# Samleo8/RadarSLAMPy

Measured on AMD Instinct MI355X. Metric: radar scan-pairs/sec (400x3768 polar), higher is better.
Workload: dtype u8/f32/f64

## Files before the change

radarslampy_amd/csrc/engine.hip:

```cpp
#include "roam_internal.h"
#include "retrack.h"
#include "kabsch_body.inc"
#include <algorithm>
#include <new>

#define KS ROAM_MAX_FEATURES
#define CART_CENTER 1012.0
#define M_PER_PX 0.0864
#define N_RETRACK 60
#define ROT_THR 0.2
#define TRANS_THR_SQ 4.0
#define ERR_THR 10.0f
#define TWO_PI 6.283185307179586476925286766559

#define RES_RING 8
enum { ST_PEAKS = 0, ST_WARP, ST_PYR, ST_KLT, ST_GRAPH, ST_CLIQUE, ST_KABSCH, ST_LM, ST_GLUE, ST_RETRACK, ST_COUNT };
static const char *kStageNames[ST_COUNT] = {"ingest_peaks", "warp_quantise", "pyramid", "klt", "consistency_graph",
                                            "max_clique", "kabsch", "mds_lm", "glue", "retrack"};

struct Engine {
    roam_engine_cfg cfg;
    int B = 0, W = 0, stage_cap = 0;
    PyrDesc pd;
    size_t rec_bytes = 0;
// ... 35 lines not shown
    int lm_big_slot = 0;
    roam_lane_result *results = nullptr;
    roam_lane_result *results_host = nullptr;
    hipEvent_t ev_res[8] = {nullptr, nullptr, nullptr, nullptr, nullptr, nullptr, nullptr, nullptr};
    hipEvent_t ev_pool = nullptr;
    bool pool_dirty = false;
    RtArgs rt;
    bool rt_on = false;
    int rt_mode = 1;
    uint8_t *kfb = nullptr;
    uint8_t *rmap = nullptr;
    int rmap_cap = 0;
    int64_t rmap_n = 0;
    int64_t rmap_n_bcast = 0;
    std::vector<int32_t> rmap_root;
    uint8_t *kfx_send = nullptr, *kfx_recv = nullptr;
    size_t kfx_rec = 0;
    int kfx_peaks = 0;
    int kfx_world = 0;
    int64_t *rmap_n_dev = nullptr;
    int32_t *rmap_root_dev = nullptr;
    int64_t kfx_calls = 0;
    bool kfx_ready = false;
    hipStream_t st_comm = nullptr;
    hipEvent_t ev_kfx[3] = {};
    int kfx_last = -1;
    hipEvent_t ev[ST_COUNT + 1] = {};
    bool stage_ev_forced = false;
    bool stage_ev = true;
    hipEvent_t ev_join = nullptr, ev_pk0 = nullptr, ev_pk1 = nullptr;
    hipEvent_t ev_klt[4] = {}, ev_g4[4] = {};
    hipEvent_t ev_warp = nullptr;
    hipEvent_t ev_idx = nullptr, ev_peaks = nullptr;
    hipEvent_t tr_ev[64][6] = {};
    hipEvent_t rt_ev[64][3 * RT_TRACE_CHUNKS] = {};
    bool rt_ev_ok[64] = {};
    hipEvent_t ev_emit = nullptr;
    RtSide det_side = {};
    int det_chunk() const { return (det_side.chunk > 0 && retrack_sided(rt, B, &det_side)) ? det_side.chunk : rt.slots; }
    int64_t rt_image_px = 0;
    bool tr_ev_ok[64] = {};
    int64_t stage_ev_step = -1;
    bool tr_ok = false;
    unsigned long long *pyr_dark = nullptr;
    static constexpr bool warp_dark_zero = true;
    bool ev_ok = false, stepped = false, uploads_pending = false;
    uint64_t up_seq = 0, up_waited = 0;
    std::vector<uint64_t> slot_seq;
    hipEvent_t ev_up_ring[16] = {};
    std::vector<int> lane_k;
    int rt_floor = 320;
    int kmax() const { int m = rt_on ? rt_floor : 64; for (int k : lane_k) m = k > m ? k : m; m = (m + 63) & ~63; return m > KS ? KS : m; }
    std::vector<void *> allocs;
};

template <typename T>
static bool dalloc(roam_ctx *ctx, Engine *e, T **p, size_t count)
{
    void *q = nullptr;
    size_t bytes = count * sizeof(T);
    if (bytes == 0) bytes = 16;
    hipError_t err = hipMalloc(&q, bytes);
    if (err != hipSuccess) {
        ROAM_SET_ERR(ctx, "engine: hipMalloc(%zu) failed: %s", bytes, hipGetErrorString(err));
        return false;
    }
// ... 135 lines not shown
        Ti[3] = s * ko[0] + c * ko[2]; Ti[4] = s * ko[1] + c * ko[3]; Ti[5] = s * hx + c * hy + y;
        Ti[6] = 0; Ti[7] = 0; Ti[8] = 1;
    }
}


#define MAP_SLOT (8 + 2 * KS)
__device__ __forceinline__ void map_freeze(double *__restrict__ map_store, int32_t *__restrict__ map_n, int map_cap, int b,
                                           const double *__restrict__ kfp, const double *__restrict__ kfv, int n,
                                           int scan, const double *__restrict__ locals)
{
    const int slot = map_n[b];
    if (slot >= map_cap) return;
    double *d = map_store + ((size_t)b * map_cap + slot) * MAP_SLOT;
    for (int j = threadIdx.x; j < 2 * n; j += blockDim.x) d[8 + j] = locals[j];
    if (threadIdx.x == 0) {
        d[0] = kfp[0]; d[1] = kfp[1]; d[2] = kfp[2];
        d[3] = kfv[0]; d[4] = kfv[1]; d[5] = kfv[2];
        d[6] = (double)n; d[7] = (double)scan;
    }
}

__global__ __launch_bounds__(256) void map_freeze_kernel(double *__restrict__ map_store, int32_t *__restrict__ map_n, int map_cap,
                                                         int b, const double *__restrict__ kf_pose,
                                                         const double *__restrict__ kf_vel, const int32_t *__restrict__ feat_n,
                                                         const int32_t *__restrict__ kf_scan, const double *__restrict__ kf_und,
                                                         const int32_t *__restrict__ kf_live, const int32_t *__restrict__ kf_fresh)
{
    if (!kf_live[b] || kf_fresh[b]) return;
    const int slot = map_n[b];
    map_freeze(map_store, map_n, map_cap, b, kf_pose + 3 * b, kf_vel + 3 * b, feat_n[b], kf_scan[b], kf_und + (size_t)b * KS * 2);
    __syncthreads();
    if (threadIdx.x == 0 && slot < map_cap) map_n[b] = slot + 1;
}

__global__ __launch_bounds__(256) void g4_update_kernel(roam_engine_cfg cfg, const double *__restrict__ lm_out,
                                                        const int32_t *__restrict__ lm_nfev, const int32_t *__restrict__ lm_info,
                                                        const double *__restrict__ kab_out, double *__restrict__ pose,
                                                        double *__restrict__ vel, double *__restrict__ kf_pose,
                                                        double *__restrict__ kf_und, const double *__restrict__ kf_und_tmp,
                                                        const double *__restrict__ p_jt, const int32_t *__restrict__ in_n,
                                                        const int32_t *__restrict__ good_n, int32_t *__restrict__ feat_n,
                                                        const int32_t *__restrict__ peaks_n, const int32_t *__restrict__ cq_flags,
                                                        roam_lane_result *__restrict__ res, const int32_t *__restrict__ scan_idx,
                                                        double *__restrict__ kf_vel, int32_t *__restrict__ kf_scan,
                                                        int32_t *__restrict__ kf_fresh, const int32_t *__restrict__ kf_live,
                                                        double *__restrict__ map_store, int32_t *__restrict__ map_n, int map_cap,
                                                        int collect, int32_t *__restrict__ rt_lane, int32_t *__restrict__ rt_scan,
                                                        int32_t *__restrict__ rt_n)
{
    __shared__ double np_[3], nv_[3];
    __shared__ int newkf;
    const int b = blockIdx.x, t = threadIdx.x;
    const int n = in_n[b];
    if (t == 0) {
        double px = pose[3 * b], py = pose[3 * b + 1], pth = pose[3 * b + 2];
        double v0 = 0, v1 = 0, v2 = 0;
        const double *k = kab_out + 6 * (int64_t)b;
        if (n >= 2) {
            if (cfg.motion_distortion) {
                const double *s = lm_out + 6 * (int64_t)b;
                v0 = s[0]; v1 = s[1]; v2 = s[2]; px = s[3]; py = s[4]; pth = s[5];
            } else {
                const double dx = k[4] * M_PER_PX, dy = k[5] * M_PER_PX, dth = atan2(k[2], k[0]);
                const double c = cos(pth), s = sin(pth);
                px += dx * c - dy * s; py += dx * s + dy * c; pth += dth;
// ... 25 lines not shown
        if (newkf) {
            const double x = p_jt[2 * o], y = p_jt[2 * o + 1];
            const double dT = 0.25 * atan2(-y, -x) / TWO_PI;
            const double a = v2 * dT, ca = cos(a), sa = sin(a);
            kf_und[2 * o] = ca * x - sa * y + v0 * dT;
            kf_und[2 * o + 1] = sa * x + ca * y + v1 * dT;
        } else {
            kf_und[2 * o] = kf_und_tmp[2 * o]; kf_und[2 * o + 1] = kf_und_tmp[2 * o + 1];
        }
    }
    __syncthreads();
    if (t == 0) {
        pose[3 * b] = np_[0]; pose[3 * b + 1] = np_[1]; pose[3 * b + 2] = np_[2];
        vel[3 * b] = v0; vel[3 * b + 1] = v1; vel[3 * b + 2] = v2;
        if (newkf) {
            kf_pose[3 * b] = np_[0]; kf_pose[3 * b + 1] = np_[1]; kf_pose[3 * b + 2] = np_[2];
            kf_vel[3 * b] = v0; kf_vel[3 * b + 1] = v1; kf_vel[3 * b + 2] = v2;
            kf_scan[b] = scan_idx[b];
            if (mslot >= 0 && mslot < map_cap) map_n[b] = mslot + 1;
        }
        kf_fresh[b] = newkf;
        feat_n[b] = n;
    }
    if (collect) {
        __shared__ int last_s, sh[4], base_s;
#if defined(__HIP_DEVICE_COMPILE__) && !defined(__gfx942__) && !defined(__gfx950__)
#error "g4_update_kernel's hand-off to its last block relies on gfx94x/95x storing with write-through and counting stores in vmcnt: s_waitcnt vmcnt(0) + relaxed atomics, no release/acquire pair"
#endif
        asm volatile("s_waitcnt vmcnt(0)" ::: "memory");
        __syncthreads();
        if (t == 0) last_s = atomicAdd(rt_n + 1, 1) == (int)gridDim.x - 1;
        __syncthreads();
        if (!last_s) return;
        const int B = (int)gridDim.x;
        if (t == 0) base_s = 0;
        __syncthreads();
        for (int b0 = 0; b0 < B; b0 += 256) {
            const int bb = b0 + t;
            const int f = (bb < B && (collect == 2 || (__hip_atomic_load(&res[bb].flags, __ATOMIC_RELAXED, __HIP_MEMORY_SCOPE_AGENT) & 4))) ? 1 : 0;
            const int lane = t & 63, w = t >> 6;
            int inc = f;
#pragma unroll
            for (int d = 1; d < 64; d <<= 1) { const int nn = __shfl_up(inc, d); if (lane >= d) inc += nn; }
            if (lane == 63) sh[w] = inc;
            __syncthreads();
            int off = base_s, tot = 0;
            for (int i = 0; i < 4; i++) { if (i < w) off += sh[i]; tot += sh[i]; }
            if (f) { rt_lane[off + inc - 1] = bb; rt_scan[off + inc - 1] = scan_idx[bb]; }
            __syncthreads();
            if (t == 0) base_s += tot;
            __syncthreads();
        }
        if (t == 0) { rt_n[0] = base_s; rt_n[1] = 0; }
    }
}

__global__ void lane_kf_reset_kernel(const float *__restrict__ feat, int K, const double *__restrict__ vel,
                                     double *__restrict__ kf_und)
{
    const int j = blockIdx.x * blockDim.x + threadIdx.x;
    if (j >= K) return;
    const double x = ((double)feat[2 * j] - CART_CENTER) * M_PER_PX, y = ((double)feat[2 * j + 1] - CART_CENTER) * M_PER_PX;
    const double dT = 0.25 * atan2(-y, -x) / TWO_PI;
    const double a = vel[2] * dT, ca = cos(a), sa = sin(a);
    kf_und[2 * j] = ca * x - sa * y + vel[0] * dT;
    kf_und[2 * j + 1] = sa * x + ca * y + vel[1] * dT;
}

#define KFB_HDR 64
#define KFB_LOCALS_OFF KFB_HDR
#define KFB_PEAKS_OFF (KFB_HDR + KS * 16)
__global__ __launch_bounds__(256) void kf_pack_kernel(uint8_t *__restrict__ buf, int lane, const double *__restrict__ kf_pose,
                                                      const double *__restrict__ kf_vel, const int32_t *__restrict__ feat_n,
                                                      const int32_t *__restrict__ kf_scan, const double *__restrict__ kf_und,
                                                      const int32_t *__restrict__ peaks_n, const int32_t *__restrict__ peaks,
                                                      int peaks_cap)
{
    const int t = blockIdx.x * blockDim.x + threadIdx.x, nt = gridDim.x * blockDim.x;
    int n = feat_n[lane], P = peaks_n[lane];
    if (n > KS) n = KS;
    if (P > peaks_cap) P = peaks_cap;
    if (t == 0) {
        roam_keyframe_hdr *h = reinterpret_cast<roam_keyframe_hdr *>(buf);
        for (int i = 0; i < 3; i++) { h->pose[i] = kf_pose[3 * lane + i]; h->velocity[i] = kf_vel[3 * lane + i]; }
        h->n_features = n; h->n_peaks = P; h->scan = kf_scan[lane]; h->lane = lane;
// ... 56 lines not shown
    }
    __syncthreads();
    if (threadIdx.x == 0) *n_dev = cnt;
}

typedef uint32_t u32x4_a1 __attribute__((ext_vector_type(4), aligned(1)));
__global__ __launch_bounds__(256) void ingest_rows_kernel(const uint8_t *__restrict__ host, int64_t host_stride, uint8_t *__restrict__ pool,
                                                          int64_t rec_bytes, int rows, int stride, int width)
{
    const int rec = blockIdx.y, row = blockIdx.x * 4 + (threadIdx.x >> 6), lane = threadIdx.x & 63;
    if (row >= rows) return;
    const uint8_t *s = host + (int64_t)rec * host_stride + (int64_t)row * stride;
    uint8_t *d = pool + (int64_t)rec * rec_bytes + (int64_t)row * stride;
    const int nvec = width / 16;
    for (int v = lane; v < nvec; v += 64) *reinterpret_cast<u32x4_a1 *>(d + 16 * v) = *reinterpret_cast<const u32x4_a1 *>(s + 16 * v);
    for (int b = nvec * 16 + lane; b < width; b += 64) d[b] = s[b];
}

extern "C" {

int32_t roam_engine_destroy(roam_ctx *ctx)
{
    if (!ctx) return ROAM_E_ARG;
    Engine *e = ctx->engine;
    if (!e) return ROAM_OK;
    hipSetDevice(ctx->device);
    hipStreamSynchronize(ctx->stream);
    for (void *p : e->allocs) hipFree(p);
    auto kill = [](hipEvent_t &ev) { if (ev) { hipEventDestroy(ev); ev = nullptr; } };
    for (auto &ev : e->ev) kill(ev);
    for (int i = 0; i < 4; i++) { kill(e->det_side.ev_i[i]); kill(e->det_side.ev_d[i]); }
    kill(e->ev_emit);
    kill(e->ev_join); kill(e->ev_pk0); kill(e->ev_pk1); kill(e->ev_warp); kill(e->ev_idx); kill(e->ev_peaks);
    for (int i = 0; i < 4; i++) { kill(e->ev_klt[i]); kill(e->ev_g4[i]); }
    for (auto &row : e->tr_ev) for (auto &ev : row) kill(ev);
    for (auto &row : e->rt_ev) for (auto &ev : row) kill(ev);
    if (e->scan_host) hipHostFree(e->scan_host);
    if (e->results_host) hipHostFree(e->results_host);
    for (auto &ev : e->ev_res) if (ev) hipEventDestroy(ev);
    if (e->st_comm) { hipStreamSynchronize(e->st_comm); hipStreamDestroy(e->st_comm); }
    for (auto &ev : e->ev_kfx) if (ev) hipEventDestroy(ev);
    if (e->ev_pool) hipEventDestroy(e->ev_pool);
    for (auto &ev : e->ev_up_ring) if (ev) hipEventDestroy(ev);
    hipStreamSynchronize(ctx->stream2);
    hipStreamSynchronize(ctx->stream4);
    delete e;
    ctx->engine = nullptr;
    return ROAM_OK;
}

static int32_t fused_tables(roam_ctx *ctx, Engine *e)
{
    RtArgs &r = e->rt;
    if (r.fd_mapT) return ROAM_OK;
    const size_t npx = (size_t)e->W * e->W, R = (size_t)r.slots;
    uint32_t *mapT = nullptr, *boxtab = nullptr, *darktab = nullptr;
    bool ok = dalloc(ctx, e, &mapT, npx) && dalloc(ctx, e, &boxtab, retrack_fused_boxtab_words(e->W)) && dalloc(ctx, e, &darktab, retrack_darktab_words(e->W));
    ok = ok && dalloc(ctx, e, &r.fd_halo, R * 2 * (size_t)r.fd_halo_words) && dalloc(ctx, e, &r.fd_cc, R * 2048);
    if (!ok) return ROAM_E_HIP;
    HIP_TRY(ctx, launch_retrack_fused_tables(ctx->stream, e->warp_map, e->W, e->cfg.clip, mapT, boxtab, darktab));
    HIP_TRY(ctx, hipStreamSynchronize(ctx->stream));
    r.fd_boxtab = boxtab; r.fd_darktab = darktab;
    r.fd_mapT = mapT;
    return ROAM_OK;
}

// ... 106 lines not shown
        }
        const size_t D = (size_t)B;
        ok = ok && dalloc(ctx, e, &r.cand_rc, D * BP_MAX_PTS) && dalloc(ctx, e, &r.cand_val, D * BP_MAX_PTS) && dalloc(ctx, e, &r.cand_n, D);
        ok = ok && dalloc(ctx, e, &r.tasks, D * BP_MAX_TASKS) && dalloc(ctx, e, &r.pairs, D * (BP_MAX_PAIRS + 1));
        ok = ok && dalloc(ctx, e, &r.order, D * (BP_MAX_PAIRS + 1)) && dalloc(ctx, e, &r.ovbits, D * ((BP_MAX_PAIRS + 31) / 32 + 1));
        ok = ok && dalloc(ctx, e, &r.bigtab, D * 2 * 131072);
        ok = ok && dalloc(ctx, e, &r.kp, D * BP_MAX_PTS * 3) && dalloc(ctx, e, &r.kp_n, D) && dalloc(ctx, e, &r.slot_flags, D);
        ok = ok && dalloc(ctx, e, &r.ssc_work, D * 4 * BP_MAX_PTS) && dalloc(ctx, e, &r.sel, D * BP_MAX_PTS) && dalloc(ctx, e, &r.sel_n, D) && dalloc(ctx, e, &r.blob_order_buf, D);
    }
    if (!ok) { roam_engine_destroy(ctx); return ROAM_E_HIP; }
    if (e->rt_on) {
        if (hipError_t er = retrack_init(); er != hipSuccess) {
            ROAM_SET_ERR(ctx, "retrack_init failed: %s", hipGetErrorString(er));
            roam_engine_destroy(ctx);
            return ROAM_E_HIP;
        }
        RtArgs &r = e->rt;
        r.pool = e->pool; r.map = e->warp_map; r.feat = e->feat; r.feat_n = e->feat_n; r.vel = e->vel; r.kf_und = e->kf_und; r.res = nullptr;
    }
    for (auto &ev : e->ev_res)
        if (hipEventCreateWithFlags(&ev, hipEventDisableTiming) != hipSuccess) { ROAM_SET_ERR(ctx, "hipEventCreate failed"); roam_engine_destroy(ctx); return ROAM_E_HIP; }
    e->slot_seq.assign((size_t)cfg->pool_scans, 0);
    for (auto &ev : e->ev_up_ring)
        if (hipEventCreateWithFlags(&ev, hipEventDisableTiming) != hipSuccess) { ROAM_SET_ERR(ctx, "hipEventCreate failed"); roam_engine_destroy(ctx); return ROAM_E_HIP; }
    if (hipEventCreateWithFlags(&e->ev_pool, hipEventDisableTiming) != hipSuccess) {
        ROAM_SET_ERR(ctx, "hipEventCreate failed"); roam_engine_destroy(ctx); return ROAM_E_HIP;
    }
    for (auto &ev : e->ev) {
        if (hipEventCreate(&ev) != hipSuccess) { ROAM_SET_ERR(ctx, "hipEventCreate failed"); roam_engine_destroy(ctx); return ROAM_E_HIP; }
    }
    if (hipEventCreate(&e->ev_join) != hipSuccess ||
        hipEventCreate(&e->ev_pk0) != hipSuccess || hipEventCreate(&e->ev_pk1) != hipSuccess ||
        hipEventCreateWithFlags(&e->ev_warp, hipEventDisableTiming) != hipSuccess || hipEventCreateWithFlags(&e->ev_idx, hipEventDisableTiming) != hipSuccess ||
        hipEventCreateWithFlags(&e->ev_peaks, hipEventDisableTiming) != hipSuccess) {
        ROAM_SET_ERR(ctx, "hipEventCreate failed"); roam_engine_destroy(ctx); return ROAM_E_HIP;
    }
    for (int i = 0; i < 4; i++)
        if (hipEventCreateWithFlags(&e->ev_klt[i], hipEventDisableTiming) != hipSuccess || hipEventCreateWithFlags(&e->ev_g4[i], hipEventDisableTiming) != hipSuccess) {
            ROAM_SET_ERR(ctx, "hipEventCreate failed"); roam_engine_destroy(ctx); return ROAM_E_HIP;
        }
    e->ev_ok = true;
    e->tr_ok = true;
    HIP_TRY(ctx, launch_warp_map(ctx->stream, cfg->rows, cfg->clip, e->warp_map));
    HIP_TRY(ctx, launch_pyr_dark(ctx->stream, e->warp_map, e->W, e->W, cfg->clip, e->pyr_dark));
    if (e->rt_on) HIP_TRY(ctx, launch_retrack_boxtab(ctx->stream, e->warp_map, e->W, cfg->clip, const_cast<uint32_t *>(e->rt.boxtab)));
    if (e->rt_on) HIP_TRY(ctx, launch_retrack_darktab(ctx->stream, e->warp_map, e->W, cfg->clip, const_cast<uint32_t *>(e->rt.darktab)));
    if (e->rt_on && e->rt.fused) { const int32_t rc_ = fused_tables(ctx, e); if (rc_ != ROAM_OK) { roam_engine_destroy(ctx); return rc_; } }
    HIP_TRY(ctx, hipStreamSynchronize(ctx->stream));
    e->rt_image_px = (int64_t)e->W * e->W;
    if (e->rt_on && e->W <= 2048 && B >= RT_TWO_PASS_SLOTS) {
        e->rt_image_px = 0;
        const size_t npx = (size_t)e->W * e->W, ndt = retrack_darktab_words(e->W), nph = retrack_phase_words(e->W);
        uint32_t *stage = nullptr;
        HIP_TRY(ctx, hipHostMalloc(reinterpret_cast<void **>(&stage), (npx + ndt + nph) * 4, hipHostMallocDefault));
        uint32_t *mh = stage, *dh = stage + npx;
        std::vector<uint32_t> ph(nph, 0u);
        hipError_t ec = hipMemcpyAsync(mh, e->warp_map, npx * 4, hipMemcpyDeviceToHost, ctx->stream);
        if (ec == hipSuccess) ec = hipMemcpyAsync(dh, e->rt.darktab, ndt * 4, hipMemcpyDeviceToHost, ctx->stream);
        if (ec == hipSuccess) ec = hipStreamSynchronize(ctx->stream);
        bool okp = ec == hipSuccess && retrack_build_phases(mh, dh, e->W, cfg->clip, ph.data());
        if (okp) {
            memcpy(stage + npx + ndt, ph.data(), nph * 4);
            ec = hipMemcpyAsync(const_cast<uint32_t *>(e->rt.phlist), stage + npx + ndt, nph * 4, hipMemcpyHostToDevice, ctx->stream);
            if (ec == hipSuccess) ec = hipStreamSynchronize(ctx->stream);
        }
        (void)hipHostFree(stage);
        if (!okp || ec != hipSuccess) { ROAM_SET_ERR(ctx, "retrack: phase list (%s)", ec != hipSuccess ? hipGetErrorString(ec) : "image too large"); roam_engine_destroy(ctx); return ec != hipSuccess ? ROAM_E_HIP : ROAM_E_ARG; }
// ... 492 lines not shown
    HIP_TRY(ctx, hipEventRecord(e->ev_warp, sA));
    HIP_TRY(ctx, hipStreamWaitEvent(sB, e->ev_warp, 0));
    if (e->ev_emit) HIP_TRY(ctx, hipStreamWaitEvent(sB, e->ev_emit, 0));
    if (e->stage_ev) HIP_TRY(ctx, hipEventRecord(tr[3], sB));
    HIP_TRY(ctx, launch_build_pyramid(sB, next, e->pd, B, e->pyr_dark));
    if (e->stage_ev) HIP_TRY(ctx, hipEventRecord(tr[4], sB));
    HIP_TRY(ctx, hipEventRecord(e->ev_join, sB));
    HIP_TRY(ctx, hipStreamWaitEvent(st, e->ev_join, 0));
    if (e->stage_ev) HIP_TRY(ctx, hipEventRecord(e->ev[ST_KLT], st));
    if (any_new) {
        hipLaunchKernelGGL(new_sequence_kernel, dim3((B + 255) / 256), dim3(256), 0, st, e->feat_n, e->scan_idx[pb] + B, B);
        HIP_TRY(ctx, hipGetLastError());
    }
    HIP_TRY(ctx, launch_klt(st, prev, next, e->pd, e->feat, e->feat_n, KM, KS, B, e->klt_next, e->klt_status, e->klt_err));
    HIP_TRY(ctx, hipEventRecord(e->ev_klt[k4], st));
    hipLaunchKernelGGL(g1_good_kernel, dim3(B), dim3(256), 0, st, e->feat, e->feat_n, e->klt_next, e->klt_status, e->klt_err,
                       e->good_old, e->good_new, e->good_idx, e->good_n, KM);
    HIP_TRY(ctx, hipGetLastError());
    if (e->stage_ev) HIP_TRY(ctx, hipEventRecord(e->ev[ST_GRAPH], st));
    if (c.reject_outliers) {
        HIP_TRY(ctx, launch_consistency_graph(st, e->good_old, e->good_new, e->good_n, KM, KS, B, 0.5 / M_PER_PX, e->adj, nw));
        if (e->stage_ev) HIP_TRY(ctx, hipEventRecord(e->ev[ST_CLIQUE], st));
        HIP_TRY(ctx, launch_max_clique(st, e->adj, e->good_n, KM, KS, nw, B, c.clique_node_limit, e->cq_stack, e->cq_mask, e->cq_n, e->cq_flags, e->cq_order));
    } else {
        if (e->stage_ev) HIP_TRY(ctx, hipEventRecord(e->ev[ST_CLIQUE], st));
        hipLaunchKernelGGL(fill_mask_kernel, dim3(B), dim3(256), 0, st, e->cq_mask, e->good_n, e->cq_n, e->cq_flags);
        HIP_TRY(ctx, hipGetLastError());
    }
    if (e->stage_ev) HIP_TRY(ctx, hipEventRecord(e->ev[ST_KABSCH], st));
    hipLaunchKernelGGL(g2_inliers_kernel, dim3(B), dim3(256), 0, st, e->good_old, e->good_new, e->good_idx, e->good_n, e->cq_mask,
                       e->kf_pose, e->kf_und, e->kf_und_tmp, e->kab_src, e->kab_tgt, e->p_w, e->p_jt, e->feat, e->in_n, e->kab_out, e->pose,
                       c.motion_distortion ? e->T_wj0 : nullptr, e->T_init);
    HIP_TRY(ctx, hipGetLastError());
    if (e->stage_ev) HIP_TRY(ctx, hipEventRecord(e->ev[ST_LM], st));
    if (c.motion_distortion) {
        MdsProblemDesc P;
        P.T_wj0 = e->T_wj0; P.T_init = e->T_init; P.p_w = e->p_w; P.p_jt = e->p_jt; P.count = e->in_n;
        P.N = KM; P.nstride = KS; P.nmax = KM; P.B = B; P.period = 0.25;
        for (int i = 0; i < 5; i++) P.sigma5[i] = c.sigma5[i];
        P.big = e->lm_big; P.big_slot = e->lm_big_slot; e->lm_big_slot ^= 1;
        HIP_TRY(ctx, launch_mds_solve(st, P, e->lm_work, e->lm_out, e->lm_nfev, e->lm_info, nullptr, nullptr));
    }
    if (e->stage_ev) HIP_TRY(ctx, hipEventRecord(e->ev[ST_GLUE], st));
    HIP_TRY(ctx, hipStreamWaitEvent(st, e->ev_peaks, 0));
    hipLaunchKernelGGL(g4_update_kernel, dim3(B), dim3(256), 0, st, c, e->lm_out, e->lm_nfev, e->lm_info, e->kab_out, e->pose,
                       e->vel, e->kf_pose, e->kf_und, e->kf_und_tmp, e->p_jt, e->in_n, e->good_n, e->feat_n, e->peaks_n[pb],
                       e->cq_flags, res_slot, e->scan_idx[pb], e->kf_vel, e->kf_scan, e->kf_fresh, e->kf_live, e->map_store, e->map_n,
                       e->map_cap, (e->rt_on && e->rt_mode) ? (e->rt_mode == 2 ? 2 : 1) : 0, e->rt.rt_lane, e->rt.rt_scan, e->rt.rt_n);
    HIP_TRY(ctx, hipGetLastError());
    if (e->stage_ev) HIP_TRY(ctx, hipEventRecord(e->ev[ST_RETRACK], st));
    if (e->rt_on && e->rt_mode) {
        e->rt.res = res_slot;
        if (B >= 256 && !e->ev_emit) HIP_TRY(ctx, hipEventCreateWithFlags(&e->ev_emit, hipEventDisableTiming));
        if (e->det_side.chunk > 0 && !e->det_side.ev_i[0]) {
            e->det_side.st = sB;
            for (int i = 0; i < 4; i++) { HIP_TRY(ctx, hipEventCreateWithFlags(&e->det_side.ev_i[i], hipEventDisableTiming)); HIP_TRY(ctx, hipEventCreateWithFlags(&e->det_side.ev_d[i], hipEventDisableTiming)); }
        }
        HIP_TRY(ctx, launch_retrack(st, e->rt, B, e->stage_ev ? e->rt_ev[e->nstep & 63] : nullptr, RT_TRACE_CHUNKS, e->ev_emit,
                                    e->det_side.chunk > 0 ? &e->det_side : nullptr));
        if (e->rt_mode == 2) e->rt_floor = std::min(KS, e->kmax() + 256);
    }
    e->rt_ev_ok[e->nstep & 63] = e->rt_on && e->rt_mode && e->stage_ev;
    if (e->stage_ev) HIP_TRY(ctx, hipEventRecord(e->ev[ST_COUNT], st));
    HIP_TRY(ctx, hipEventRecord(e->ev_g4[k4], st));
    HIP_TRY(ctx, hipMemcpyAsync(e->results_host + (size_t)rs * B, res_slot, sizeof(roam_lane_result) * (size_t)B, hipMemcpyDeviceToHost, st));
    HIP_TRY(ctx, hipEventRecord(e->ev_res[rs], st));
    e->cur = (e->cur + 1) & 3;
    e->pk = pb;
    e->nstep++;
    e->stepped = true;
    return ROAM_OK;
}

int32_t roam_engine_results(roam_ctx *ctx, roam_lane_result *out, int32_t n)
{
    ENGINE();
    ARG_CHECK(ctx, out && n >= 1 && n <= e->B);
    if (e->nstep == 0) { ROAM_SET_ERR(ctx, "no step enqueued"); return ROAM_E_STATE; }
    return roam_engine_step_results(ctx, e->nstep - 1, out, n);
}

int32_t roam_engine_step_results(roam_ctx *ctx, int64_t step, roam_lane_result *out, int32_t n)
{
    ENGINE();
    ARG_CHECK(ctx, out && n >= 1 && n <= e->B);
    if (step < 0 || step >= e->nstep || step < e->nstep - RES_RING) {
        ROAM_SET_ERR(ctx, "step %lld is not in the result ring (steps %lld..%lld)", (long long)step,
                     (long long)std::max<int64_t>(0, e->nstep - RES_RING), (long long)e->nstep - 1);
        return ROAM_E_STATE;
    }
    const int rs = (int)(step % RES_RING);
    HIP_TRY(ctx, hipEventSynchronize(e->ev_res[rs]));
// ... 71 lines not shown
int32_t roam_engine_lane_image(roam_ctx *ctx, int32_t lane, int32_t level, uint8_t *out, int64_t cap)
{
    ENGINE();
    ARG_CHECK(ctx, lane >= 0 && lane < e->B && level >= 0 && level < ROAM_PYR_LEVELS && out);
    const size_t n = (size_t)e->pd.w[level] * e->pd.h[level];
    ARG_CHECK(ctx, cap >= (int64_t)n);
    HIP_TRY(ctx, hipMemcpyAsync(out, e->pyr[e->cur] + (size_t)lane * e->pd.lane_stride + e->pd.off[level], n,
                                hipMemcpyDeviceToHost, ctx->stream));
    HIP_TRY(ctx, hipStreamSynchronize(ctx->stream));
    return ROAM_OK;
}

int32_t roam_engine_set_stage_events(roam_ctx *ctx, int32_t on)
{
    ENGINE();
    if (!e->stage_ev_forced) e->stage_ev = on != 0;
    return ROAM_OK;
}

int32_t roam_engine_stage_times(roam_ctx *ctx, float *ms_out, const char **names_out, int32_t cap, int32_t *n)
{
    ENGINE();
    ARG_CHECK(ctx, ms_out && n && cap >= ST_COUNT);
    if (!e->stepped) { ROAM_SET_ERR(ctx, "no step recorded"); return ROAM_E_STATE; }
    if (!e->stage_ev) { ROAM_SET_ERR(ctx, "stage events are off (roam_engine_set_stage_events)"); return ROAM_E_STATE; }
    if (e->stage_ev_step != e->nstep - 1) { ROAM_SET_ERR(ctx, "the last step was enqueued with stage events off: run a step first"); return ROAM_E_STATE; }
    HIP_TRY(ctx, hipStreamSynchronize(ctx->stream));
    for (int i = 0; i < ST_COUNT; i++) {
        float ms = 0;
        hipEvent_t *tl = e->tr_ev[(e->nstep - 1) & 63];
        if (i == ST_PEAKS) HIP_TRY(ctx, hipEventElapsedTime(&ms, tl[0], tl[5]));
        else if (i == ST_WARP) HIP_TRY(ctx, hipEventElapsedTime(&ms, tl[1], tl[2]));
        else if (i == ST_PYR) HIP_TRY(ctx, hipEventElapsedTime(&ms, tl[3], tl[4]));
        else HIP_TRY(ctx, hipEventElapsedTime(&ms, e->ev[i], e->ev[i + 1]));
        ms_out[i] = ms;
        if (names_out) names_out[i] = kStageNames[i];
    }
    *n = ST_COUNT;
    return ROAM_OK;
}

int32_t roam_engine_kernel_avg(roam_ctx *ctx, const char *name, int32_t last_steps, float *avg_ms, int32_t *n_used)
{
    ENGINE();
    ARG_CHECK(ctx, name && last_steps >= 1 && avg_ms && n_used);
    if (!e->stage_ev) { ROAM_SET_ERR(ctx, "stage events are off (roam_engine_set_stage_events)"); return ROAM_E_STATE; }
    int k = !strcmp(name, "ingest_peaks") ? 0 : (!strcmp(name, "warp_quantise") ? 1 : (!strcmp(name, "pyramid") ? 2 : -1));
    const int kd = !strcmp(name, "doh_integral") ? 0 : (!strcmp(name, "doh_det_maxima") ? 1 : -1);
    if (k < 0 && kd < 0) { ROAM_SET_ERR(ctx, "unknown kernel '%s'", name); return ROAM_E_ARG; }
    if (kd >= 0 && !e->rt_on) { ROAM_SET_ERR(ctx, "engine created without retrack_on_device"); return ROAM_E_STATE; }
    if (!e->stepped) { ROAM_SET_ERR(ctx, "run a step first"); return ROAM_E_STATE; }
    HIP_TRY(ctx, hipStreamSynchronize(ctx->stream));
    int64_t n = std::min<int64_t>(std::min<int64_t>(last_steps, e->nstep), 64);
    double sum = 0;
    if (kd >= 0) {
        int64_t used = 0;
        for (int64_t i = e->nstep - n; i < e->nstep; i++) {
            if (!e->rt_ev_ok[i & 63]) continue;
            float ms = 0;
            HIP_TRY(ctx, hipEventElapsedTime(&ms, e->rt_ev[i & 63][kd], e->rt_ev[i & 63][kd + 1]));
            sum += ms; used++;
        }
        *avg_ms = used ? (float)(sum / (double)used) : 0.f;
        *n_used = (int32_t)used;
        return ROAM_OK;
    }
// ... 144 lines not shown
```

radarslampy_amd/csrc/retrack.h:

```cpp
#pragma once
#include "roam_internal.h"
#include "blobprune.h"

#define RT_TWO_PASS_SLOTS 200
enum { RT_F_CAND_OVERFLOW = 1, RT_F_TREE_OVERFLOW = 2, RT_F_PAIR_OVERFLOW = 4, RT_F_FEAT_OVERFLOW = 8 };

struct RtArgs {
    int W, rows, cols, stride, payload_off, slots, size1, size2;
    int64_t rec_bytes;
    double sigma1, sigma2, threshold;
    const uint8_t *pool;
    const uint32_t *map;
    const uint32_t *phlist;
    const uint32_t *boxtab;
    const uint32_t *darktab;
    float *feat;
    int32_t *feat_n;
    const double *vel;
    double *kf_und;
    roam_lane_result *res;
    int32_t *rt_n, *rt_lane, *rt_scan;
    double *S;
    int32_t *col_done;
    double *colT;
    int SP;
    uint32_t *cand_rc;
    double *cand_val;
    int32_t *cand_n;
    BpTask *tasks;
    uint32_t *pairs;
    uint16_t *order;
    uint32_t *ovbits;
    uint16_t *bigtab;
    double *kp;
    int32_t *kp_n, *slot_flags;
    int32_t *ssc_work;
    int32_t *sel, *sel_n;
    int32_t *blob_order_buf;
    const int32_t *blob_order;
    int fused;
    const uint32_t *fd_mapT;
    const uint32_t *fd_boxtab;
    const uint32_t *fd_darktab;
    double *fd_halo;
    int64_t fd_halo_words;
    double *fd_cc;
};

hipError_t launch_retrack_collect(hipStream_t st, const roam_lane_result *res, const int32_t *scan_idx, int B, int force_all, const RtArgs &a);
#define RT_TRACE_CHUNKS 16
struct RtSide { hipStream_t st; hipEvent_t ev_i[4], ev_d[4]; int chunk; };
bool retrack_sided(const RtArgs &a, int B, const RtSide *side);
hipError_t launch_retrack(hipStream_t st, const RtArgs &a, int B, hipEvent_t *trace = nullptr, int ntrace = 0, hipEvent_t after_order = nullptr, const RtSide *side = nullptr);
hipError_t launch_ssc_batch(hipStream_t st, const double *kp, int64_t kp_stride, const int32_t *count, int kp_cap, int P,
                            int num_ret, double tol, int cols, int rows, int32_t *work, int32_t *sel, int32_t *n_sel,
                            const int32_t *n_active, int first);
hipError_t launch_retrack_part(hipStream_t st, const RtArgs &a, int P, int which);
hipError_t launch_retrack_emit(hipStream_t st, const RtArgs &a, int P);
hipError_t retrack_init();
size_t retrack_boxtab_words(int W);
size_t retrack_phase_words(int W);
int retrack_band_rows();
bool retrack_build_phases(const uint32_t *map_host, const uint32_t *darktab_host, int W, int cols, uint32_t *out);
hipError_t launch_retrack_boxtab(hipStream_t st, const uint32_t *map, int W, int cols, uint32_t *boxtab);
size_t retrack_darktab_words(int W);
size_t retrack_fused_boxtab_words(int W);
size_t retrack_fused_halo_words(int W);
hipError_t launch_retrack_fused_tables(hipStream_t st, const uint32_t *map, int W, int cols, uint32_t *mapT, uint32_t *boxtab, uint32_t *darktab);
hipError_t launch_retrack_darktab(hipStream_t st, const uint32_t *map, int W, int cols, uint32_t *darktab);
```

radarslampy_amd/csrc/retrack.hip:

```cpp
#include "roam_internal.h"
#include "doh_common.h"
#include "blobprune.h"
#include "npsort_wave.h"
#include "retrack.h"
#include <algorithm>

#define KS ROAM_MAX_FEATURES
#define CART_CENTER 1012.0
#define M_PER_PX 0.0864
#define TWO_PI 6.283185307179586476925286766559

__global__ __launch_bounds__(256) void rt_collect_kernel(const roam_lane_result *__restrict__ res, const int32_t *__restrict__ scan_idx,
                                                         int B, int force_all, int32_t *__restrict__ rt_lane,
                                                         int32_t *__restrict__ rt_scan, int32_t *__restrict__ rt_n)
{
    __shared__ int sh[8];
    __shared__ int base_s;
    const int t = threadIdx.x;
    if (t == 0) base_s = 0;
    __syncthreads();
    for (int b0 = 0; b0 < B; b0 += 256) {
        const int b = b0 + t;
        const int f = (b < B && (force_all || (res[b].flags & 4))) ? 1 : 0;
        const int lane = t & 63, w = t >> 6;
// ... 1618 lines not shown
        }
    }
    if (!sound) {
        n = 0;
        for (int b = 0; b < nbands; b++)
            for (int g = 0; g < RI_GROUPS && g * 64 * RI_WAVES < W; g++) out[1 + n++] = (uint32_t)b | ((uint32_t)g << 8) | (((1u << RI_WAVES) - 1u) << 12);
    }
    out[0] = (uint32_t)n;
    return true;
}

hipError_t retrack_init()
{
    if (hipError_t ef = hipFuncSetAttribute(reinterpret_cast<const void *>(rt_fused_kernel), hipFuncAttributeMaxDynamicSharedMemorySize, FD_LDS_BYTES); ef != hipSuccess) return ef;
    hipError_t e = hipFuncSetAttribute(reinterpret_cast<const void *>(rt_det_strip_kernel), hipFuncAttributeMaxDynamicSharedMemorySize, SD_LDS_BYTES);
    if (e != hipSuccess) return e;
    return hipFuncSetAttribute(reinterpret_cast<const void *>(rt_integral_kernel), hipFuncAttributeMaxDynamicSharedMemorySize, RI_LDS_BYTES);
}

static hipError_t launch_det(hipStream_t st, const RtArgs &a, int first, int P)
{
    const int W = a.W;
    if (a.size1 != 15 || a.size2 != 30) return hipErrorInvalidValue;
    const int ns = (W + SD_OUT - 1) / SD_OUT;
    hipLaunchKernelGGL(rt_det_strip_kernel, dim3((unsigned)(((int64_t)P * ns + 7) / 8 * 8)), dim3(SD_THREADS), SD_LDS_BYTES, st, a, first, P, ns);
    return hipGetLastError();
}

bool retrack_sided(const RtArgs &a, int B, const RtSide *side)
{
    return side && side->chunk > 0 && a.W <= 2048 && !a.fused && a.slots >= 2 * side->chunk && B > side->chunk;
}

hipError_t launch_retrack(hipStream_t st, const RtArgs &a, int B, hipEvent_t *trace, int ntrace, hipEvent_t after_order, const RtSide *side)
{
    const int W = a.W, R = a.slots;
    hipError_t e = hipSuccess;
    const bool sided = retrack_sided(a, B, side);
    if (sided) {
        const int C = side->chunk;
        int nc = 0;
        for (int first = 0; first < B; first += C, nc++) {
            const int P = min(C, B - first);
            const bool tr = trace && nc < ntrace;
            hipEvent_t *tev = trace + 3 * nc;
            RtArgs ac = a;
            ac.S = a.S + (size_t)(nc & 1) * C * a.SP * W;
            if (nc >= 2 && (e = hipStreamWaitEvent(st, side->ev_d[(nc - 2) & 3], 0)) != hipSuccess) return e;
            if (tr && (e = hipEventRecord(tev[0], st)) != hipSuccess) return e;
            if (B - first >= RI_MIN_DETECTIONS) hipLaunchKernelGGL(rt_integral_kernel, dim3(P), dim3(64 * (RI_WAVES + 1)), RI_LDS_BYTES, st, ac, first);
            const int P2 = min(P, RT_TWO_PASS_SLOTS);
            hipLaunchKernelGGL(rt_integ_cols_kernel, dim3((W + 63) / 64, (W + RC_BAND - 1) / RC_BAND, min(P2, RT_TWO_PASS_Z)), dim3(256), 0, st, ac, first, P2);
            hipLaunchKernelGGL(rt_integ_rows_kernel, dim3((W + RR_ROWS - 1) / RR_ROWS, min(P2, RT_TWO_PASS_Z)), dim3(256), 0, st, ac, first, P2);
            if ((e = hipGetLastError()) != hipSuccess) return e;
            if (tr && (e = hipEventRecord(tev[1], st)) != hipSuccess) return e;
            if ((e = hipEventRecord(side->ev_i[nc & 3], st)) != hipSuccess) return e;
            if ((e = hipStreamWaitEvent(side->st, side->ev_i[nc & 3], 0)) != hipSuccess) return e;
            if ((e = launch_det(side->st, ac, first, P)) != hipSuccess) return e;
            if (tr && (e = hipEventRecord(tev[2], side->st)) != hipSuccess) return e;
            if ((e = hipEventRecord(side->ev_d[nc & 3], side->st)) != hipSuccess) return e;
        }
        for (int k = max(0, nc - 2); k < nc; k++)
            if ((e = hipStreamWaitEvent(st, side->ev_d[k & 3], 0)) != hipSuccess) return e;
    } else
    for (int first = 0; first < B; first += R) {
        const int P = min(R, B - first);
        const bool tr = trace && first / R < ntrace;
        hipEvent_t *tev = trace + 3 * (first / R);
        if (tr && (e = hipEventRecord(tev[0], st)) != hipSuccess) return e;
        if (W <= 2048 && a.fused && B - first >= RI_MIN_DETECTIONS) hipLaunchKernelGGL(rt_fused_kernel, dim3(P), dim3(FD_THREADS), FD_LDS_BYTES, st, a, first, 0);
        else if (W <= 2048 && B - first >= RI_MIN_DETECTIONS)
            hipLaunchKernelGGL(rt_integral_kernel, dim3(P), dim3(64 * (RI_WAVES + 1)), RI_LDS_BYTES, st, a, first);
        if ((e = hipGetLastError()) != hipSuccess) return e;
        const int P2 = min(P, RT_TWO_PASS_SLOTS);
        hipLaunchKernelGGL(rt_integ_cols_kernel, dim3((W + 63) / 64, (W + RC_BAND - 1) / RC_BAND, min(P2, RT_TWO_PASS_Z)), dim3(256), 0, st, a, first, P2);
        hipLaunchKernelGGL(rt_integ_rows_kernel, dim3((W + RR_ROWS - 1) / RR_ROWS, min(P2, RT_TWO_PASS_Z)), dim3(256), 0, st, a, first, P2);
        if ((e = hipGetLastError()) != hipSuccess) return e;
        if (tr && (e = hipEventRecord(tev[1], st)) != hipSuccess) return e;
        if ((e = launch_det(st, a, first, P)) != hipSuccess) return e;
        if (tr && (e = hipEventRecord(tev[2], st)) != hipSuccess) return e;
    }
    if (B < 256) {
        RtArgs ab = a;
        ab.blob_order = nullptr;
        hipLaunchKernelGGL(rt_book_kernel, dim3(B), dim3(64), 0, st, ab, 0);
        if ((e = hipGetLastError()) != hipSuccess) return e;
    } else {
        hipLaunchKernelGGL(rt_emit_kernel, dim3(B), dim3(256), 0, st, a, 0);
        RtArgs ab = a;
        ab.blob_order = nullptr;
        if (B >= 512 && a.blob_order_buf) {
            if ((e = launch_order_by_count(st, a.cand_n, B, BP_MAX_PTS, a.blob_order_buf, 1)) != hipSuccess) return e;
            ab.blob_order = a.blob_order_buf;
        }
        if (after_order && (e = hipEventRecord(after_order, st)) != hipSuccess) return e;
        hipLaunchKernelGGL(rt_blobs_kernel<true>, dim3(B), dim3(64), 0, st, ab, 0);
        hipLaunchKernelGGL(rt_blobs_kernel<false>, dim3(B), dim3(64), 0, st, ab, 0);
        e = launch_ssc_batch(st, a.kp, (int64_t)BP_MAX_PTS * 3, a.kp_n, BP_MAX_PTS, B, 200, 0.1, W, W, a.ssc_work, a.sel, a.sel_n, a.rt_n, 0);
        if (e != hipSuccess) return e;
    }
    hipLaunchKernelGGL(rt_append_kernel, dim3(B), dim3(256), 0, st, a, 0);
    return hipGetLastError();
}

hipError_t launch_retrack_collect(hipStream_t st, const roam_lane_result *res, const int32_t *scan_idx, int B, int force_all, const RtArgs &a)
{
    hipLaunchKernelGGL(rt_collect_kernel, dim3(1), dim3(256), 0, st, res, scan_idx, B, force_all, a.rt_lane, a.rt_scan, a.rt_n);
    return hipGetLastError();
}

hipError_t launch_retrack_emit(hipStream_t st, const RtArgs &a, int P)
{
    hipLaunchKernelGGL(rt_emit_kernel, dim3(P), dim3(256), 0, st, a, 0);
    return hipGetLastError();
}

hipError_t launch_retrack_part(hipStream_t st, const RtArgs &a_in, int P, int which)
{
    RtArgs a = a_in;
    a.fused = which >= 2 ? 1 : 0;
    const int W = a.W;
    if (which >= 2) {
        if (!a.fd_mapT) return hipErrorInvalidValue;
        hipLaunchKernelGGL(rt_fused_kernel, dim3(P), dim3(FD_THREADS), FD_LDS_BYTES, st, a, 0, which - 2);
        return hipGetLastError();
    }
    if (which == 0) {
        hipLaunchKernelGGL(rt_integral_kernel, dim3(P), dim3(64 * (RI_WAVES + 1)), RI_LDS_BYTES, st, a, 0);
        const int P2 = min(P, RT_TWO_PASS_SLOTS);
        hipLaunchKernelGGL(rt_integ_cols_kernel, dim3((W + 63) / 64, (W + RC_BAND - 1) / RC_BAND, min(P2, RT_TWO_PASS_Z)), dim3(256), 0, st, a, 0, P2);
        hipLaunchKernelGGL(rt_integ_rows_kernel, dim3((W + RR_ROWS - 1) / RR_ROWS, min(P2, RT_TWO_PASS_Z)), dim3(256), 0, st, a, 0, P2);
    } else {
        return launch_det(st, a, 0, P);
// ... 4 lines not shown
```

Baseline: 54000.

## Overlap retrack detection with LM solve and glue on a side stream

```diff
diff --git a/radarslampy_amd/csrc/engine.hip b/radarslampy_amd/csrc/engine.hip
--- a/radarslampy_amd/csrc/engine.hip
+++ b/radarslampy_amd/csrc/engine.hip
@@ -91,6 +91,9 @@
     hipEvent_t ev_klt[4] = {}, ev_g4[4] = {};
     hipEvent_t ev_warp = nullptr;
     hipEvent_t ev_idx = nullptr, ev_peaks = nullptr;
+    hipEvent_t ev_fork = nullptr, ev_side = nullptr;
+    hipEvent_t ev_glue1 = nullptr;
+    bool stage_side = false;
     hipEvent_t tr_ev[64][6] = {};
     hipEvent_t rt_ev[64][3 * RT_TRACE_CHUNKS] = {};
     bool rt_ev_ok[64] = {};
@@ -292,6 +295,39 @@
     map_freeze(map_store, map_n, map_cap, b, kf_pose + 3 * b, kf_vel + 3 * b, feat_n[b], kf_scan[b], kf_und + (size_t)b * KS * 2);
     __syncthreads();
     if (threadIdx.x == 0 && slot < map_cap) map_n[b] = slot + 1;
+}
+
+template <typename F>
+__device__ __forceinline__ void rt_list_block(int B, F flagged, const int32_t *__restrict__ scan_idx, int32_t *__restrict__ rt_lane,
+                                              int32_t *__restrict__ rt_scan, int *sh, int *base_s)
+{
+    const int t = threadIdx.x;
+    if (t == 0) *base_s = 0;
+    __syncthreads();
+    for (int b0 = 0; b0 < B; b0 += 256) {
+        const int bb = b0 + t;
+        const int f = (bb < B && flagged(bb)) ? 1 : 0;
+        const int lane = t & 63, w = t >> 6;
+        int inc = f;
+#pragma unroll
+        for (int d = 1; d < 64; d <<= 1) { const int nn = __shfl_up(inc, d); if (lane >= d) inc += nn; }
+        if (lane == 63) sh[w] = inc;
+        __syncthreads();
+        int off = *base_s, tot = 0;
+        for (int i = 0; i < 4; i++) { if (i < w) off += sh[i]; tot += sh[i]; }
+        if (f) { rt_lane[off + inc - 1] = bb; rt_scan[off + inc - 1] = scan_idx[bb]; }
+        __syncthreads();
+        if (t == 0) *base_s += tot;
+        __syncthreads();
+    }
+}
+
+__global__ __launch_bounds__(256) void rt_list_kernel(const int32_t *__restrict__ in_n, const int32_t *__restrict__ scan_idx, int B, int all,
+                                                      int32_t *__restrict__ rt_lane, int32_t *__restrict__ rt_scan, int32_t *__restrict__ rt_n)
+{
+    __shared__ int sh[4], base_s;
+    rt_list_block(B, [&](int bb) { return all || in_n[bb] <= N_RETRACK; }, scan_idx, rt_lane, rt_scan, sh, &base_s);
+    if (threadIdx.x == 0) rt_n[0] = base_s;
 }
 
 __global__ __launch_bounds__(256) void g4_update_kernel(roam_engine_cfg cfg, const double *__restrict__ lm_out,
@@ -383,25 +419,8 @@
         if (t == 0) last_s = atomicAdd(rt_n + 1, 1) == (int)gridDim.x - 1;
         __syncthreads();
         if (!last_s) return;
-        const int B = (int)gridDim.x;
-        if (t == 0) base_s = 0;
-        __syncthreads();
-        for (int b0 = 0; b0 < B; b0 += 256) {
-            const int bb = b0 + t;
-            const int f = (bb < B && (collect == 2 || (__hip_atomic_load(&res[bb].flags, __ATOMIC_RELAXED, __HIP_MEMORY_SCOPE_AGENT) & 4))) ? 1 : 0;
-            const int lane = t & 63, w = t >> 6;
-            int inc = f;
-#pragma unroll
-            for (int d = 1; d < 64; d <<= 1) { const int nn = __shfl_up(inc, d); if (lane >= d) inc += nn; }
-            if (lane == 63) sh[w] = inc;
-            __syncthreads();
-            int off = base_s, tot = 0;
-            for (int i = 0; i < 4; i++) { if (i < w) off += sh[i]; tot += sh[i]; }
-            if (f) { rt_lane[off + inc - 1] = bb; rt_scan[off + inc - 1] = scan_idx[bb]; }
-            __syncthreads();
-            if (t == 0) base_s += tot;
-            __syncthreads();
-        }
+        rt_list_block((int)gridDim.x, [&](int bb) { return collect == 2 || (__hip_atomic_load(&res[bb].flags, __ATOMIC_RELAXED, __HIP_MEMORY_SCOPE_AGENT) & 4); },
+                      scan_idx, rt_lane, rt_scan, sh, &base_s);
         if (t == 0) { rt_n[0] = base_s; rt_n[1] = 0; }
     }
 }
@@ -524,6 +543,7 @@
     for (int i = 0; i < 4; i++) { kill(e->det_side.ev_i[i]); kill(e->det_side.ev_d[i]); }
     kill(e->ev_emit);
     kill(e->ev_join); kill(e->ev_pk0); kill(e->ev_pk1); kill(e->ev_warp); kill(e->ev_idx); kill(e->ev_peaks);
+    kill(e->ev_fork); kill(e->ev_side); kill(e->ev_glue1);
     for (int i = 0; i < 4; i++) { kill(e->ev_klt[i]); kill(e->ev_g4[i]); }
     for (auto &row : e->tr_ev) for (auto &ev : row) kill(ev);
     for (auto &row : e->rt_ev) for (auto &ev : row) kill(ev);
@@ -696,7 +716,9 @@
     if (hipEventCreate(&e->ev_join) != hipSuccess ||
         hipEventCreate(&e->ev_pk0) != hipSuccess || hipEventCreate(&e->ev_pk1) != hipSuccess ||
         hipEventCreateWithFlags(&e->ev_warp, hipEventDisableTiming) != hipSuccess || hipEventCreateWithFlags(&e->ev_idx, hipEventDisableTiming) != hipSuccess ||
-        hipEventCreateWithFlags(&e->ev_peaks, hipEventDisableTiming) != hipSuccess) {
+        hipEventCreateWithFlags(&e->ev_peaks, hipEventDisableTiming) != hipSuccess ||
+        hipEventCreateWithFlags(&e->ev_fork, hipEventDisableTiming) != hipSuccess || hipEventCreateWithFlags(&e->ev_side, hipEventDisableTiming) != hipSuccess ||
+        hipEventCreate(&e->ev_glue1) != hipSuccess) {
         ROAM_SET_ERR(ctx, "hipEventCreate failed"); roam_engine_destroy(ctx); return ROAM_E_HIP;
     }
     for (int i = 0; i < 4; i++)
@@ -1255,32 +1277,49 @@
                        e->kf_pose, e->kf_und, e->kf_und_tmp, e->kab_src, e->kab_tgt, e->p_w, e->p_jt, e->feat, e->in_n, e->kab_out, e->pose,
                        c.motion_distortion ? e->T_wj0 : nullptr, e->T_init);
     HIP_TRY(ctx, hipGetLastError());
-    if (e->stage_ev) HIP_TRY(ctx, hipEventRecord(e->ev[ST_LM], st));
+    const bool detect = e->rt_on && e->rt_mode;
+    const bool side = detect && B >= 256;
+    hipStream_t sL = side ? sP : st;
+    if (side) {
+        hipLaunchKernelGGL(rt_list_kernel, dim3(1), dim3(256), 0, st, e->in_n, e->scan_idx[pb], B, e->rt_mode == 2 ? 1 : 0, e->rt.rt_lane, e->rt.rt_scan, e->rt.rt_n);
+        HIP_TRY(ctx, hipGetLastError());
+        if (e->stage_ev) HIP_TRY(ctx, hipEventRecord(e->ev[ST_RETRACK], st));
+        HIP_TRY(ctx, hipEventRecord(e->ev_fork, st));
+        HIP_TRY(ctx, hipStreamWaitEvent(sL, e->ev_fork, 0));
+    }
+    if (e->stage_ev) HIP_TRY(ctx, hipEventRecord(e->ev[ST_LM], sL));
     if (c.motion_distortion) {
         MdsProblemDesc P;
         P.T_wj0 = e->T_wj0; P.T_init = e->T_init; P.p_w = e->p_w; P.p_jt = e->p_jt; P.count = e->in_n;
         P.N = KM; P.nstride = KS; P.nmax = KM; P.B = B; P.period = 0.25;
         for (int i = 0; i < 5; i++) P.sigma5[i] = c.sigma5[i];
         P.big = e->lm_big; P.big_slot = e->lm_big_slot; e->lm_big_slot ^= 1;
-        HIP_TRY(ctx, launch_mds_solve(st, P, e->lm_work, e->lm_out, e->lm_nfev, e->lm_info, nullptr, nullptr));
-    }
-    if (e->stage_ev) HIP_TRY(ctx, hipEventRecord(e->ev[ST_GLUE], st));
-    HIP_TRY(ctx, hipStreamWaitEvent(st, e->ev_peaks, 0));
-    hipLaunchKernelGGL(g4_update_kernel, dim3(B), dim3(256), 0, st, c, e->lm_out, e->lm_nfev, e->lm_info, e->kab_out, e->pose,
+        HIP_TRY(ctx, launch_mds_solve(sL, P, e->lm_work, e->lm_out, e->lm_nfev, e->lm_info, nullptr, nullptr));
+    }
+    if (e->stage_ev) HIP_TRY(ctx, hipEventRecord(e->ev[ST_GLUE], sL));
+    if (!side) HIP_TRY(ctx, hipStreamWaitEvent(st, e->ev_peaks, 0));
+    hipLaunchKernelGGL(g4_update_kernel, dim3(B), dim3(256), 0, sL, c, e->lm_out, e->lm_nfev, e->lm_info, e->kab_out, e->pose,
                        e->vel, e->kf_pose, e->kf_und, e->kf_und_tmp, e->p_jt, e->in_n, e->good_n, e->feat_n, e->peaks_n[pb],
                        e->cq_flags, res_slot, e->scan_idx[pb], e->kf_vel, e->kf_scan, e->kf_fresh, e->kf_live, e->map_store, e->map_n,
-                       e->map_cap, (e->rt_on && e->rt_mode) ? (e->rt_mode == 2 ? 2 : 1) : 0, e->rt.rt_lane, e->rt.rt_scan, e->rt.rt_n);
+                       e->map_cap, (detect && !side) ? (e->rt_mode == 2 ? 2 : 1) : 0, e->rt.rt_lane, e->rt.rt_scan, e->rt.rt_n);
     HIP_TRY(ctx, hipGetLastError());
-    if (e->stage_ev) HIP_TRY(ctx, hipEventRecord(e->ev[ST_RETRACK], st));
-    if (e->rt_on && e->rt_mode) {
+    if (side) {
+        if (e->stage_ev) HIP_TRY(ctx, hipEventRecord(e->ev_glue1, sL));
+        HIP_TRY(ctx, hipEventRecord(e->ev_side, sL));
+    } else if (e->stage_ev) HIP_TRY(ctx, hipEventRecord(e->ev[ST_RETRACK], st));
+    if (e->stage_ev) e->stage_side = side;
+    if (detect) {
         e->rt.res = res_slot;
         if (B >= 256 && !e->ev_emit) HIP_TRY(ctx, hipEventCreateWithFlags(&e->ev_emit, hipEventDisableTiming));
         if (e->det_side.chunk > 0 && !e->det_side.ev_i[0]) {
             e->det_side.st = sB;
             for (int i = 0; i < 4; i++) { HIP_TRY(ctx, hipEventCreateWithFlags(&e->det_side.ev_i[i], hipEventDisableTiming)); HIP_TRY(ctx, hipEventCreateWithFlags(&e->det_side.ev_d[i], hipEventDisableTiming)); }
         }
+        int n_min = 0;
+        if (e->rt_mode == 2) n_min = B;
+        else for (int b = 0; b < B; b++) n_min += (scan_idx[b] & ROAM_STEP_NEW_SEQUENCE) ? 1 : 0;
         HIP_TRY(ctx, launch_retrack(st, e->rt, B, e->stage_ev ? e->rt_ev[e->nstep & 63] : nullptr, RT_TRACE_CHUNKS, e->ev_emit,
-                                    e->det_side.chunk > 0 ? &e->det_side : nullptr));
+                                    e->det_side.chunk > 0 ? &e->det_side : nullptr, side ? e->ev_side : nullptr, n_min));
         if (e->rt_mode == 2) e->rt_floor = std::min(KS, e->kmax() + 256);
     }
     e->rt_ev_ok[e->nstep & 63] = e->rt_on && e->rt_mode && e->stage_ev;
@@ -1418,6 +1457,8 @@
         if (i == ST_PEAKS) HIP_TRY(ctx, hipEventElapsedTime(&ms, tl[0], tl[5]));
         else if (i == ST_WARP) HIP_TRY(ctx, hipEventElapsedTime(&ms, tl[1], tl[2]));
         else if (i == ST_PYR) HIP_TRY(ctx, hipEventElapsedTime(&ms, tl[3], tl[4]));
+        else if (i == ST_KABSCH && e->stage_side) HIP_TRY(ctx, hipEventElapsedTime(&ms, e->ev[ST_KABSCH], e->ev[ST_RETRACK]));
+        else if (i == ST_GLUE && e->stage_side) HIP_TRY(ctx, hipEventElapsedTime(&ms, e->ev[ST_GLUE], e->ev_glue1));
         else HIP_TRY(ctx, hipEventElapsedTime(&ms, e->ev[i], e->ev[i + 1]));
         ms_out[i] = ms;
         if (names_out) names_out[i] = kStageNames[i];
diff --git a/radarslampy_amd/csrc/retrack.h b/radarslampy_amd/csrc/retrack.h
--- a/radarslampy_amd/csrc/retrack.h
+++ b/radarslampy_amd/csrc/retrack.h
@@ -51,7 +51,8 @@
 #define RT_TRACE_CHUNKS 16
 struct RtSide { hipStream_t st; hipEvent_t ev_i[4], ev_d[4]; int chunk; };
 bool retrack_sided(const RtArgs &a, int B, const RtSide *side);
-hipError_t launch_retrack(hipStream_t st, const RtArgs &a, int B, hipEvent_t *trace = nullptr, int ntrace = 0, hipEvent_t after_order = nullptr, const RtSide *side = nullptr);
+hipError_t launch_retrack(hipStream_t st, const RtArgs &a, int B, hipEvent_t *trace = nullptr, int ntrace = 0, hipEvent_t after_order = nullptr, const RtSide *side = nullptr,
+                          hipEvent_t join = nullptr, int n_min = 0);
 hipError_t launch_ssc_batch(hipStream_t st, const double *kp, int64_t kp_stride, const int32_t *count, int kp_cap, int P,
                             int num_ret, double tol, int cols, int rows, int32_t *work, int32_t *sel, int32_t *n_sel,
                             const int32_t *n_active, int first);
diff --git a/radarslampy_amd/csrc/retrack.hip b/radarslampy_amd/csrc/retrack.hip
--- a/radarslampy_amd/csrc/retrack.hip
+++ b/radarslampy_amd/csrc/retrack.hip
@@ -1674,9 +1674,11 @@
     return side && side->chunk > 0 && a.W <= 2048 && !a.fused && a.slots >= 2 * side->chunk && B > side->chunk;
 }
 
-hipError_t launch_retrack(hipStream_t st, const RtArgs &a, int B, hipEvent_t *trace, int ntrace, hipEvent_t after_order, const RtSide *side)
+hipError_t launch_retrack(hipStream_t st, const RtArgs &a, int B, hipEvent_t *trace, int ntrace, hipEvent_t after_order, const RtSide *side,
+                          hipEvent_t join, int n_min)
 {
     const int W = a.W, R = a.slots;
+    auto two_pass = [&](int first) { return !(W <= 2048 && n_min - first >= RI_MIN_DETECTIONS); };
     hipError_t e = hipSuccess;
     const bool sided = retrack_sided(a, B, side);
     if (sided) {
@@ -1692,8 +1694,10 @@
             if (tr && (e = hipEventRecord(tev[0], st)) != hipSuccess) return e;
             if (B - first >= RI_MIN_DETECTIONS) hipLaunchKernelGGL(rt_integral_kernel, dim3(P), dim3(64 * (RI_WAVES + 1)), RI_LDS_BYTES, st, ac, first);
             const int P2 = min(P, RT_TWO_PASS_SLOTS);
-            hipLaunchKernelGGL(rt_integ_cols_kernel, dim3((W + 63) / 64, (W + RC_BAND - 1) / RC_BAND, min(P2, RT_TWO_PASS_Z)), dim3(256), 0, st, ac, first, P2);
-            hipLaunchKernelGGL(rt_integ_rows_kernel, dim3((W + RR_ROWS - 1) / RR_ROWS, min(P2, RT_TWO_PASS_Z)), dim3(256), 0, st, ac, first, P2);
+            if (two_pass(first)) {
+                hipLaunchKernelGGL(rt_integ_cols_kernel, dim3((W + 63) / 64, (W + RC_BAND - 1) / RC_BAND, min(P2, RT_TWO_PASS_Z)), dim3(256), 0, st, ac, first, P2);
+                hipLaunchKernelGGL(rt_integ_rows_kernel, dim3((W + RR_ROWS - 1) / RR_ROWS, min(P2, RT_TWO_PASS_Z)), dim3(256), 0, st, ac, first, P2);
+            }
             if ((e = hipGetLastError()) != hipSuccess) return e;
             if (tr && (e = hipEventRecord(tev[1], st)) != hipSuccess) return e;
             if ((e = hipEventRecord(side->ev_i[nc & 3], st)) != hipSuccess) return e;
@@ -1715,8 +1719,10 @@
             hipLaunchKernelGGL(rt_integral_kernel, dim3(P), dim3(64 * (RI_WAVES + 1)), RI_LDS_BYTES, st, a, first);
         if ((e = hipGetLastError()) != hipSuccess) return e;
         const int P2 = min(P, RT_TWO_PASS_SLOTS);
-        hipLaunchKernelGGL(rt_integ_cols_kernel, dim3((W + 63) / 64, (W + RC_BAND - 1) / RC_BAND, min(P2, RT_TWO_PASS_Z)), dim3(256), 0, st, a, first, P2);
-        hipLaunchKernelGGL(rt_integ_rows_kernel, dim3((W + RR_ROWS - 1) / RR_ROWS, min(P2, RT_TWO_PASS_Z)), dim3(256), 0, st, a, first, P2);
+        if (two_pass(first)) {
+            hipLaunchKernelGGL(rt_integ_cols_kernel, dim3((W + 63) / 64, (W + RC_BAND - 1) / RC_BAND, min(P2, RT_TWO_PASS_Z)), dim3(256), 0, st, a, first, P2);
+            hipLaunchKernelGGL(rt_integ_rows_kernel, dim3((W + RR_ROWS - 1) / RR_ROWS, min(P2, RT_TWO_PASS_Z)), dim3(256), 0, st, a, first, P2);
+        }
         if ((e = hipGetLastError()) != hipSuccess) return e;
         if (tr && (e = hipEventRecord(tev[1], st)) != hipSuccess) return e;
         if ((e = launch_det(st, a, first, P)) != hipSuccess) return e;
@@ -1741,6 +1747,7 @@
         e = launch_ssc_batch(st, a.kp, (int64_t)BP_MAX_PTS * 3, a.kp_n, BP_MAX_PTS, B, 200, 0.1, W, W, a.ssc_work, a.sel, a.sel_n, a.rt_n, 0);
         if (e != hipSuccess) return e;
     }
+    if (join && (e = hipStreamWaitEvent(st, join, 0)) != hipSuccess) return e;
     hipLaunchKernelGGL(rt_append_kernel, dim3(B), dim3(256), 0, st, a, 0);
     return hipGetLastError();
 }
```

After: 52710. 2.4% lower.
